# DavidHan008/SLAM-1

Measured on AMD Instinct MI355X. Metric: frames/sec tracking+local-BA @1280x720, higher is better.
Workload: dtype u8+f32+f64

## Files before the change

### slam-1_amd/csrc/ba.hip

```cpp
#include "common.hpp"

#include <cmath>

namespace {

typedef double d4 __attribute__((ext_vector_type(4)));

__device__ __forceinline__ void st_sc1(double* p, double v) {
  __hip_atomic_store(p, v, __ATOMIC_RELAXED, __HIP_MEMORY_SCOPE_AGENT);
}
__device__ __forceinline__ double ld_sc1(const double* p) {
  return __hip_atomic_load(const_cast<double*>(p), __ATOMIC_RELAXED, __HIP_MEMORY_SCOPE_AGENT);
}
__device__ __forceinline__ unsigned ticket_add(uint32_t* p) {
  return __hip_atomic_fetch_add(p, 1u, __ATOMIC_RELAXED, __HIP_MEMORY_SCOPE_AGENT);
}
__device__ __forceinline__ void ticket_reset(uint32_t* p) {
  __hip_atomic_store(p, 0u, __ATOMIC_RELAXED, __HIP_MEMORY_SCOPE_AGENT);
}

constexpr double kClamp = 5000.0;
constexpr double kDiagMin = 1e-6, kDiagMax = 1e32;
constexpr double kLamMin = 1e-16, kLamMax = 1e32;
constexpr int kBS = 256;
// ... 267 lines not shown
  if (threadIdx.x == 0) {
    const int nw = (blockDim.x + 63) >> 6;
    for (int w = 0; w < nw; ++w) s += lds[w];
  }
  __syncthreads();
  return s;
}

__global__ __launch_bounds__(kBS) void k_residual(const double* __restrict__ cams,
                                                  const double* __restrict__ pts,
                                                  const int32_t* __restrict__ ci,
                                                  const int32_t* __restrict__ pi,
                                                  const double* __restrict__ qs, int n_obs,
                                                  double* __restrict__ resid,
                                                  double* __restrict__ jac) {
  const int o = blockIdx.x * kBS + threadIdx.x;
  if (o >= n_obs) return;
  double r[2], J[2][12];
  if (jac) {
    reproject<true>(cams + 9 * ci[o], pts + 3 * pi[o], qs + 2 * o, r, J);
    clamp_rows<true>(r, J);
    for (int a = 0; a < 2; ++a)
      for (int k = 0; k < 12; ++k) jac[(size_t)o * 24 + a * 12 + k] = J[a][k];
  } else {
    reproject<false>(cams + 9 * ci[o], pts + 3 * pi[o], qs + 2 * o, r, J);
    clamp_rows<false>(r, J);
  }
  resid[2 * o] = r[0];
  resid[2 * o + 1] = r[1];
}

__device__ __forceinline__ int cur_of(const double* state) {
  return state[SLAM_BA_ST_CUR] != 0.0 ? 1 : 0;
}

__device__ __forceinline__ double clampd(double d) { return fmin(fmax(d, kDiagMin), kDiagMax); }

constexpr int kDenseMaxN = 120;
__host__ __device__ __forceinline__ bool sys_packed(int n_cams) { return 9 * n_cams > kDenseMaxN; }
__host__ __device__ __forceinline__ long long sys_vec_off(int n_cams, int n_blocks) {
  return sys_packed(n_cams) ? 81ll * n_blocks : 81ll * n_cams * n_cams;
}


struct PtSchur {
  double V00 = 0, V01 = 0, V02 = 0, V11 = 0, V12 = 0, V22 = 0, g0 = 0, g1 = 0, g2 = 0;
  double d[3], iv[6], e[3];
  __device__ __forceinline__ void acc(double j0, double j1, double j2, double rr) {
    V00 += j0 * j0; V01 += j0 * j1; V02 += j0 * j2;
    V11 += j1 * j1; V12 += j1 * j2; V22 += j2 * j2;
    g0 -= j0 * rr; g1 -= j1 * rr; g2 -= j2 * rr;
  }
  __device__ __forceinline__ void solve(double lam);
};
__device__ __forceinline__ void PtSchur::solve(double lam) {
  d[0] = clampd(V00); d[1] = clampd(V11); d[2] = clampd(V22);
  const double a00 = V00 + lam * d[0], a11 = V11 + lam * d[1], a22 = V22 + lam * d[2];
  const double a01 = V01, a02 = V02, a12 = V12;
  const double c00 = a11 * a22 - a12 * a12;
  const double c01 = a02 * a12 - a01 * a22;
  const double c02 = a01 * a12 - a02 * a11;
  const double c11 = a00 * a22 - a02 * a02;
  const double c12 = a01 * a02 - a00 * a12;
  const double c22 = a00 * a11 - a01 * a01;
  const double det = a00 * c00 + a01 * c01 + a02 * c02;
  const double id = det != 0.0 ? 1.0 / det : 0.0;
  iv[0] = c00 * id; iv[1] = c01 * id; iv[2] = c02 * id;
  iv[3] = c11 * id; iv[4] = c12 * id; iv[5] = c22 * id;
  e[0] = iv[0] * g0 + iv[1] * g1 + iv[2] * g2;
  e[1] = iv[1] * g0 + iv[3] * g1 + iv[4] * g2;
  e[2] = iv[2] * g0 + iv[4] * g1 + iv[5] * g2;
}

__device__ __forceinline__ double pt_comp(const double* jr, int stride, int kb, int ke, int j) {
  const int ia = j < 3 ? 0 : j < 5 ? 1 : j < 6 ? 2 : j - 6;
  const int ib = j < 3 ? j : j < 5 ? j - 2 : 2;
  const bool isg = j >= 6;
  const double* xr[2] = {jr + ia * stride, jr + (3 + ia) * stride};
  const double* yr[2] = {jr + (isg ? 6 : ib) * stride, jr + (isg ? 7 : 3 + ib) * stride};
  double v = 0.0;
  for (int k = kb; k < ke; k += 4) {
    double x[4][2], y[4][2];
#pragma unroll
    for (int u = 0; u < 4; ++u) {
      const int kk = min(k + u, ke - 1);
#pragma unroll
      for (int a = 0; a < 2; ++a) {
        x[u][a] = xr[a][kk];
        y[u][a] = yr[a][kk];
      }
    }
#pragma unroll
    for (int u = 0; u < 4; ++u) {
      if (k + u >= ke) break;
#pragma unroll
      for (int a = 0; a < 2; ++a) v += (isg ? -x[u][a] : x[u][a]) * y[u][a];
    }
  }
  return v;
}

constexpr int kCPart = 112;
constexpr int kGrp = 128;
constexpr int kLinWG = 256;
constexpr int kSlotLds = 128;
constexpr int kPairLds = 1024;

struct LinLds {
  double jc[kGrp][18];
  double w[kGrp][27];
  double ru[kGrp][4];
  double pt[kGrp][9];
  int lpt[kGrp];
  int cobs[kGrp];
  int cptr[kSlotLds];
  int bptr[kSlotLds];
  int pairs[kPairLds];
  unsigned fx[kGrp];
};

__device__ __forceinline__ void y_row(const double* W, const double* Vi, int i, double y[3]) {
  const double a = W[3 * i], b = W[3 * i + 1], c = W[3 * i + 2];
  y[0] = a * Vi[0] + b * Vi[1] + c * Vi[2];
  y[1] = a * Vi[1] + b * Vi[3] + c * Vi[4];
  y[2] = a * Vi[2] + b * Vi[4] + c * Vi[5];
}

__device__ __forceinline__ void lin_slots(const slam_ba_problem& p, LinLds& L, int cs0, int ncs,
                                          int bs0, int nbs, const int* cptr, int coff,
                                          const int* bptr, int boff, const int* pairs) {
  const int t = threadIdx.x;
  const int* cobs = L.cobs;
  for (int item = t; item < 9 * (ncs + nbs); item += kLinWG) {
    const int sl = item / 9, i = item - 9 * sl;
    double acc[9];
#pragma unroll
    for (int j = 0; j < 9; ++j) acc[j] = 0.0;
    if (sl < ncs) {
      const int s = cs0 + sl;
      double vr = 0.0, vu = 0.0, vd = 0.0, cost = 0.0;
      const int qb = cptr[sl] - coff, qe = cptr[sl + 1] - coff;
      int k = cobs[qb < qe ? qb : 0], lk = L.lpt[k];
      for (int q = qb; q < qe; ++q) {
        const int kn = cobs[q + 1 < qe ? q + 1 : q], lkn = L.lpt[kn];
        const double* jc = L.jc[k];
        const double* W = L.w[k];
        double y[3];
        y_row(W, L.pt[lk] + 3, i, y);
        const double a0 = jc[i], a1 = jc[9 + i];
#pragma unroll
        for (int j = 0; j < 9; ++j) {
          const double u = __builtin_fma(a0, jc[j], a1 * jc[9 + j]);
          const double v = __builtin_fma(y[0], W[3 * j], __builtin_fma(y[1], W[3 * j + 1], y[2] * W[3 * j + 2]));
          acc[j] += u - v;
        }
        const double r0 = L.ru[k][0], r1 = L.ru[k][1];
        vr = __builtin_fma(a0, r0, __builtin_fma(a1, r1, vr));
        vu = __builtin_fma(a0, L.ru[k][2], __builtin_fma(a1, L.ru[k][3], vu));
        vd = __builtin_fma(a0, a0, __builtin_fma(a1, a1, vd));
        cost = __builtin_fma(r0, r0, __builtin_fma(r1, r1, cost));
        k = kn;
        lk = lkn;
      }
      double* out = p.cpart + (size_t)p.cslot_row[s] * kCPart;
#pragma unroll
      for (int j = 0; j < 9; ++j) out[9 * i + j] = acc[j];
      out[81 + i] = vr;
      out[90 + i] = vu;
      out[99 + i] = vd;
      if (i == 0) out[108] = cost;
    } else {
      const int sb = sl - ncs, s = bs0 + sb;
      const int qb = bptr[sb] - boff, qe = bptr[sb + 1] - boff;
      int pr = pairs[qb < qe ? qb : 0], lk = L.lpt[pr & 0xffff];
      for (int q = qb; q < qe; ++q) {
        const int prn = pairs[q + 1 < qe ? q + 1 : q], lkn = L.lpt[prn & 0xffff];
        const int k1 = pr & 0xffff, k2 = pr >> 16;
        double y[3];
        y_row(L.w[k1], L.pt[lk] + 3, i, y);
        const double* W2 = L.w[k2];
#pragma unroll
        for (int j = 0; j < 9; ++j)
          acc[j] = __builtin_fma(y[0], W2[3 * j], __builtin_fma(y[1], W2[3 * j + 1], __builtin_fma(y[2], W2[3 * j + 2], acc[j])));
        pr = prn;
        lk = lkn;
      }
      double* out = p.bpart + (size_t)p.bslot_row[s] * 81;
#pragma unroll
      for (int j = 0; j < 9; ++j) out[9 * i + j] = acc[j];
    }
  }
}

#ifdef SLAM_LIN_PROFILE
#define LIN_T(i) const uint64_t lin_t##i = __builtin_amdgcn_s_memtime()
#else
#define LIN_T(i) (void)0
#endif
__global__ __launch_bounds__(kLinWG) void k_linearize(BaBatch bat) {
  BA_PROB_X(bat);
  const int g = bx;
  if (g >= p.n_grps) return;
  lm_wave_priority();
  __shared__ LinLds L;
  LIN_T(0);
  const int p0 = p.grp_ptr[g], p1 = p.grp_ptr[g + 1];
  const int o0 = p.pt_ptr[p0], o1 = p.pt_ptr[p1];
  const int t = threadIdx.x;
  const int o = o0 + t;
  const bool has = t < kGrp && o < o1;
  const int cur = cur_of(p.state);
  const int cs0 = p.grp_cslot[g], ncs = p.grp_cslot[g + 1] - cs0;
  const int bs0 = p.grp_bslot[g], nbs = p.grp_bslot[g + 1] - bs0;
  const int cb0 = p.cslot_obs_ptr[cs0], pb0 = p.bslot_pair_ptr[bs0];
  const int npairs = p.bslot_pair_ptr[bs0 + nbs] - pb0;
  const bool fit_c = ncs < kSlotLds, fit_b = nbs < kSlotLds, fit_p = npairs <= kPairLds;
  if (fit_c && t <= ncs) L.cptr[t] = p.cslot_obs_ptr[cs0 + t] - cb0;
  if (fit_b && t <= nbs) L.bptr[t] = p.bslot_pair_ptr[bs0 + t] - pb0;
  if (t < kGrp && t < o1 - o0) L.cobs[t] = p.cslot_obs[cb0 + t];
  if (fit_p)
    for (int q = t; q < npairs; q += kLinWG) L.pairs[q] = p.bslot_pairs[pb0 + q];
  double r[2], J[2][12];
  if (has) {
    const int pt = p.obs_pt[o];
    reproject_pre<true>(p.camrec[cur] + kCamRec * p.obs_cam[o], p.pts[cur] + 3 * pt,
                        p.obs_q + 2 * o, r, J);
    clamp_rows<true>(r, J);
#pragma unroll
    for (int a = 0; a < 2; ++a) {
#pragma unroll
      for (int i = 0; i < 9; ++i) L.jc[t][9 * a + i] = J[a][i];
#pragma unroll
      for (int c = 0; c < 3; ++c) L.w[t][3 * a + c] = J[a][9 + c];
      L.w[t][6 + a] = r[a];
      L.ru[t][a] = r[a];
    }
    L.lpt[t] = pt - p0;
  }
  __syncthreads();
  if (p.cam_fixed != nullptr) {
    for (int sl = t; sl < ncs; sl += kLinWG) {
      const unsigned fx = p.cam_fixed[p.cslot_cam[cs0 + sl]];
      const int qe = p.cslot_obs_ptr[cs0 + sl + 1] - cb0;
      for (int q = p.cslot_obs_ptr[cs0 + sl] - cb0; q < qe; ++q) L.fx[L.cobs[q]] = fx;
    }
    __syncthreads();
    if (has) {
      const unsigned fx = L.fx[t];
      if (fx) {
        hold_cols(J, fx);
#pragma unroll
        for (int i = 0; i < 9; ++i)
          if ((fx >> i) & 1u) L.jc[t][i] = L.jc[t][9 + i] = 0.0;
      }
    }
  }
  LIN_T(1);
  const double lam = p.state[SLAM_BA_ST_LAMBDA];
  if (t < p1 - p0) {
    const int pt = p0 + t;
    PtSchur ps;
    for (int k = p.pt_ptr[pt] - o0; k < p.pt_ptr[pt + 1] - o0; ++k) {
#pragma unroll
      for (int a = 0; a < 2; ++a) ps.acc(L.w[k][3 * a], L.w[k][3 * a + 1], L.w[k][3 * a + 2], L.w[k][6 + a]);
    }
    ps.solve(lam);
#pragma unroll
    for (int k = 0; k < 3; ++k) L.pt[t][k] = ps.e[k];
#pragma unroll
    for (int k = 0; k < 6; ++k) L.pt[t][3 + k] = ps.iv[k];
  }
  __syncthreads();
  if (has) {
    const double* e = L.pt[L.lpt[t]];
#pragma unroll
    for (int i = 0; i < 9; ++i)
#pragma unroll
      for (int c = 0; c < 3; ++c) L.w[t][3 * i + c] = J[0][i] * J[0][9 + c] + J[1][i] * J[1][9 + c];
    L.ru[t][2] = J[0][9] * e[0] + J[0][10] * e[1] + J[0][11] * e[2];
    L.ru[t][3] = J[1][9] * e[0] + J[1][10] * e[1] + J[1][11] * e[2];
  }
  __syncthreads();
  LIN_T(2);
  if (fit_c && fit_b && fit_p)
    lin_slots(p, L, cs0, ncs, bs0, nbs, L.cptr, 0, L.bptr, 0, L.pairs);
  else
    lin_slots(p, L, cs0, ncs, bs0, nbs, p.cslot_obs_ptr + cs0, cb0, p.bslot_pair_ptr + bs0, pb0,
              p.bslot_pairs + pb0);
#ifdef SLAM_LIN_PROFILE
  __builtin_amdgcn_s_waitcnt(0);
  __syncthreads();
  LIN_T(3);
  if (g == 7 && t == 0) {
    p.state[12] = (double)(lin_t1 - lin_t0);
    p.state[13] = (double)(lin_t2 - lin_t1);
    p.state[14] = (double)(lin_t3 - lin_t2);
    p.state[15] = (double)(ncs * 100 + nbs);
  }
#endif
}

constexpr int kMObs = 120, kMPts = 16, kMCams = 7, kMRows = 64;
constexpr int kMWG = 256;
constexpr int kSgMeta = 24;
constexpr int kNoObs = 255;
constexpr int kMObsS = kMObs + 1;
struct alignas(16) MLds {
  double jc[18][kMObsS];
  double jp[6][kMObsS];
  double ru[4][kMObsS];
  double vi[kMPts][6];
  double e[kMPts][3];
  double yt[kMPts][3][kMRows];
  double wt[kMPts][3][kMRows];
  double cam[kMCams][kCamRec];
  double X[kMPts][3];
  double zero;
  int optr[kMPts + 1];
  int lpt[kMObs];
  int la[kMObs];
  int cobs[kMObs];
  int cptr[8];
  uint8_t kfirst[kMPts][8];
  unsigned fx[kMCams];
  int crow[kMCams];
  int bab[kMCams * (kMCams - 1) / 2], brow[kMCams * (kMCams - 1) / 2];
};
static_assert(sizeof(MLds) <= 80 * 1024, "k_lin_mfma: two workgroups per CU");
static_assert(offsetof(MLds, ru) == offsetof(MLds, jp) + 6 * kMObsS * sizeof(double),
              "k_lin_mfma: (B) reads Jp and r as the rows of one array");
static_assert(kMObs <= kNoObs && kMCams <= 8 && kMPts * 8 <= kMWG, "k_lin_mfma: kfirst");
static_assert(16 * kMPts <= kMWG && 2 * kMCams <= 16, "k_lin_mfma: 16 lanes per point in (B), (C)");
static_assert(9 * kMCams <= kMRows, "k_lin_mfma: 9m rows in 4 tile rows");
static_assert(kMCams * kCamRec + kMCams <= kMWG, "k_lin_mfma: a lane per record entry and per mask word");
static_assert(2 * kMPts * 3 * kMRows >= kMRows * kMRows + kMCams * 256, "staging aliases yt/wt");

#ifdef SLAM_LINM_PROFILE
__device__ unsigned long long g_linm_stamp[4096][8];
#define LINM_DECL() unsigned long long linm_prev = __builtin_amdgcn_s_memtime(), linm_acc[7] = {0, 0, 0, 0, 0, 0, 0}
#define LINM_T(i)                                                  \
  do {                                                             \
    if (threadIdx.x == 0) {                                        \
      const unsigned long long linm_now = __builtin_amdgcn_s_memtime(); \
      linm_acc[i] += linm_now - linm_prev;                         \
      linm_prev = linm_now;                                        \
    }                                                              \
  } while (0)
#define LINM_END()                                                               \
  do {                                                                           \
    if (threadIdx.x == 0 && blockIdx.x + 1024 * blockIdx.y < 4096)               \
      for (int linm_i = 0; linm_i < 7; ++linm_i)                                 \
        g_linm_stamp[blockIdx.x + 1024 * blockIdx.y][linm_i] = linm_acc[linm_i]; \
  } while (0)
#else
#define LINM_DECL() (void)0
#define LINM_T(i) (void)0
#define LINM_END() (void)0
#endif

struct AsmTab {
  const int32_t* need;
  int32_t* cnt;
  const int32_t* cam_dblk;
  const int32_t* row_blk;
  int n_empty;
  const int32_t* empty;
  __device__ explicit AsmTab(const slam_ba_problem& p) {
    const int nb = p.n_blocks;
    need = p.asm_tab;
    cnt = p.asm_tab + nb;
    cam_dblk = p.asm_tab + 2 * nb;
    row_blk = cam_dblk + p.n_cams;
    n_empty = row_blk[p.n_bslots];
    empty = row_blk + p.n_bslots + 1;
  }
};

__device__ void fold_rows_sum(const double* __restrict__ part, int stride, int rb, int re, int n,
                              double* red, double* out) {
  const int t = threadIdx.x;
  const int nparts = kMWG / n, k = t / n, e = t - k * n;
  if (k < nparts) {
    double a[4] = {0.0, 0.0, 0.0, 0.0};
    int r = rb + k;
    for (; r + 3 * nparts < re; r += 4 * nparts) {
      double v[4];
#pragma unroll
      for (int u = 0; u < 4; ++u) v[u] = ld_sc1(part + (size_t)(r + u * nparts) * stride + e);
#pragma unroll
      for (int u = 0; u < 4; ++u) a[u] += v[u];
    }
    for (int u = 0; r < re; r += nparts, ++u) a[u] += ld_sc1(part + (size_t)r * stride + e);
    red[k * n + e] = (a[0] + a[1]) + (a[2] + a[3]);
  }
  __syncthreads();
  if (t < n) {
    double v = 0.0;
    for (int q = 0; q < nparts; ++q) v += red[q * n + t];
    out[t] = v;
  }
  __syncthreads();
}

__device__ void fold_block(const slam_ba_problem& p, int blk, double* scratch) {
  double* red = scratch;
  double* sh = scratch + 3 * kCPart;
  double* sb = sh + kCPart;
  const int c1 = p.blocks[2 * blk], c2 = p.blocks[2 * blk + 1];
  const int C9 = 9 * p.n_cams, t = threadIdx.x;
  double* S = p.sys;
  double* bvec = S + sys_vec_off(p.n_cams, p.n_blocks);
  double* gvec = bvec + C9;
  double* diagU = gvec + C9;
  double* costc = diagU + C9;
  const bool diag = c1 == c2;
  const int bb = p.blk_bslot_ptr[blk], be = p.blk_bslot_ptr[blk + 1];
  if (diag) fold_rows_sum(p.cpart, kCPart, p.cam_cslot_ptr[c1], p.cam_cslot_ptr[c1 + 1], 109, red, sh);
  if (be > bb) {
    fold_rows_sum(p.bpart, 81, bb, be, 81, red, sb);
  } else if (t < 81) {
    sb[t] = 0.0;
  }
  __syncthreads();
  if (sys_packed(p.n_cams)) {
    if (t < 81) S[(size_t)blk * 81 + t] = diag ? sh[t] - (sb[t] + sb[9 * (t % 9) + t / 9]) : -sb[t];
  } else if (t < 81) {
    const int i = t / 9, j = t - 9 * (t / 9);
    if (diag) {
      S[(size_t)(9 * c1 + i) * C9 + 9 * c1 + j] = sh[t] - (sb[t] + sb[9 * j + i]);
    } else {
      S[(size_t)(9 * c1 + i) * C9 + 9 * c2 + j] = -sb[t];
      S[(size_t)(9 * c2 + j) * C9 + 9 * c1 + i] = -sb[t];
    }
  }
  if (diag && t < 9) {
    gvec[9 * c1 + t] = -sh[81 + t];
    bvec[9 * c1 + t] = -sh[81 + t] - sh[90 + t];
    diagU[9 * c1 + t] = sh[99 + t];
  }
  if (diag && t == 0) costc[c1] = sh[108];
  __syncthreads();
}

__device__ void fold_zero_block(const slam_ba_problem& p, int blk, int t0, int nt) {
  const int c1 = p.blocks[2 * blk], c2 = p.blocks[2 * blk + 1];
  const int C9 = 9 * p.n_cams;
  double* S = p.sys;
  double* bvec = S + sys_vec_off(p.n_cams, p.n_blocks);
  for (int e = t0; e < 81; e += nt) {
    const int i = e / 9, j = e - 9 * (e / 9);
    if (sys_packed(p.n_cams)) {
      S[(size_t)blk * 81 + e] = 0.0;
    } else {
      S[(size_t)(9 * c1 + i) * C9 + 9 * c2 + j] = 0.0;
      S[(size_t)(9 * c2 + j) * C9 + 9 * c1 + i] = 0.0;
    }
  }
  if (c1 == c2)
    for (int e = t0; e < 28; e += nt) {
      if (e < 27) bvec[(size_t)(e / 9) * C9 + 9 * c1 + e % 9] = 0.0;
      else bvec[3 * (size_t)C9 + c1] = 0.0;
    }
}

__device__ void lin_fold_assemble(const slam_ba_problem& p, const int* cams, int m, int nb,
                                  const int* brow, double* scratch) {
  const AsmTab A(p);
  __shared__ int done[kMCams + kMCams * (kMCams - 1) / 2];
  __shared__ int ndone;
  __builtin_amdgcn_s_waitcnt(0);
  __syncthreads();
  if (threadIdx.x == 0) {
    int n = 0;
    for (int q = 0; q < m + nb; ++q) {
      const int blk = q < m ? A.cam_dblk[cams[q]] : A.row_blk[brow[q - m]];
      const int old = (int)ticket_add(reinterpret_cast<uint32_t*>(A.cnt + blk));
      if (old == A.need[blk] - 1) {
        done[n++] = blk;
        __hip_atomic_store(A.cnt + blk, 0, __ATOMIC_RELAXED, __HIP_MEMORY_SCOPE_AGENT);
      }
    }
    ndone = n;
  }
  __syncthreads();
  for (int q = 0; q < ndone; ++q) fold_block(p, done[q], scratch);
}

__global__ __launch_bounds__(kMWG) void k_lin_mfma(BaBatch bat) {
  BA_PROB_X(bat);
  const int sg = bx;
  if (sg >= p.n_sgrps) return;
  LINM_DECL();
  lm_wave_priority();
  __shared__ MLds L;
  if (p.asm_tab != nullptr) {
    const AsmTab A(p);
    for (int q = sg; q < A.n_empty; q += p.n_sgrps) fold_zero_block(p, A.empty[q], threadIdx.x, kMWG);
  }
  const int t = threadIdx.x, lane = t & 63;
  const int wid = __builtin_amdgcn_readfirstlane(t >> 6);
  const int* sm = p.sg_meta + kSgMeta * sg;
  const int ch0 = sm[0], ch1 = sm[1], cs0 = sm[2], m = sm[3], bs0 = sm[4], nb = sm[5];
  const int nt = (9 * m + 15) >> 4;
  const int cur = cur_of(p.state);
  const double lam = p.state[SLAM_BA_ST_LAMBDA];
  const bool held = p.cam_fixed != nullptr;
  if (t < kMCams * kCamRec) {
    const int a = t / kCamRec, k = t - kCamRec * (t / kCamRec);
    const int c = a < m ? sm[10 + a] : -1;
    if (c >= 0) L.cam[a][k] = p.camrec[cur][(size_t)kCamRec * c + k];
  } else if (held && t - kMCams * kCamRec < m) {
    const int a = t - kMCams * kCamRec;
    L.fx[a] = p.cam_fixed[sm[10 + a]];
  }
  if (t == 0) L.zero = 0.0;
  if (t < m) L.crow[t] = p.cslot_row[cs0 + t];
  if (t >= 64 && t - 64 < nb) {
    L.bab[t - 64] = p.bslot_ab[bs0 + t - 64];
    L.brow[t - 64] = p.bslot_row[bs0 + t - 64];
  }
  int tI[3], tJ[3];
  int ntl = 0;
  {
    int s = 0;
    for (int I = 0; I < nt; ++I)
      for (int J = I; J < nt; ++J, ++s)
        if ((s & 3) == wid && ntl < 3) {
          tI[ntl] = I;
          tJ[ntl] = J;
          ++ntl;
        }
  }
  const int nza = (m > wid) + (m > wid + 4);
  int tRow[3], tCol[3];
#pragma unroll
  for (int s = 0; s < 3; ++s) {
    tRow[s] = 16 * (s < ntl ? tI[s] : 0) + (lane & 15);
    tCol[s] = 16 * (s < ntl ? tJ[s] : 0) + (lane & 15);
  }
  d4 acc[3], zacc[2];
#pragma unroll
  for (int s = 0; s < 3; ++s) acc[s] = d4{0.0, 0.0, 0.0, 0.0};
#pragma unroll
  for (int s = 0; s < 2; ++s) zacc[s] = d4{0.0, 0.0, 0.0, 0.0};
  const int mi = lane & 15, mk = lane >> 4;

  struct ChunkIn {
    double q0, q1, xv;
    int meta, pp, cp;
  };
  auto load_in = [&](int ch, int p0, int p1, int o0, int o1) {
    ChunkIn in{0.0, 0.0, 0.0, 0, 0, 0};
    const int nobs = o1 - o0, npts = p1 - p0;
    const int ko = t & 127;
    if (ko < nobs) {
      in.q0 = p.obs_q[2 * (o0 + ko)];
      in.q1 = p.obs_q[2 * (o0 + ko) + 1];
    }
    if (t < nobs) in.meta = p.obs_meta[o0 + t];
    if (t < 3 * npts) in.xv = p.pts[cur][3 * p0 + t];
    if (t >= 128 && t - 128 <= npts) in.pp = p.pt_ptr[p0 + t - 128] - o0;
    if (t < 8) in.cp = p.chk_cptr[8 * ch + t];
    return in;
  };
  int p0 = sm[6], p1 = sm[7], o0 = sm[8], o1 = sm[9];
  int np0 = 0, np1 = 0, no0 = 0, no1 = 0;
  if (ch0 + 1 < ch1) {
    np0 = p.grp_ptr[ch0 + 1];
    np1 = p.grp_ptr[ch0 + 2];
    no0 = p.chk_optr[ch0 + 1];
    no1 = p.chk_optr[ch0 + 2];
  }
  ChunkIn in = load_in(ch0, p0, p1, o0, o1);
  {
    typedef double dbl2 __attribute__((ext_vector_type(2)));
    dbl2* y2 = reinterpret_cast<dbl2*>(&L.yt[0][0][0]);
    dbl2* w2 = reinterpret_cast<dbl2*>(&L.wt[0][0][0]);
    for (int i = t; i < kMPts * 3 * kMRows / 2; i += kMWG) {
      y2[i] = dbl2{0.0, 0.0};
      w2[i] = dbl2{0.0, 0.0};
    }
  }
  for (int ch = ch0; ch < ch1; ++ch) {
    const int nobs = o1 - o0, npts = p1 - p0;
    const double q0 = in.q0, q1 = in.q1;
    __syncthreads();
    if (t < nobs) {
      L.lpt[t] = in.meta & 255;
      L.la[t] = (in.meta >> 8) & 255;
      L.cobs[t] = in.meta >> 16;
    }
    if (t < 3 * npts) (&L.X[0][0])[t] = in.xv;
    if (t >= 128 && t - 128 <= npts) L.optr[t - 128] = in.pp;
    if (t < 8) L.cptr[t] = in.cp;
    int tl = t;
    asm volatile("" : "+v"(tl));
    if (tl < kMPts * 8) (&L.kfirst[0][0])[tl] = kNoObs;
    __syncthreads();
    if (tl < nobs && (tl == 0 || L.lpt[tl - 1] != L.lpt[tl] || L.la[tl - 1] != L.la[tl]))
      L.kfirst[L.lpt[tl]][L.la[tl]] = (uint8_t)tl;
    int nnp0 = 0, nnp1 = 0, nno0 = 0, nno1 = 0;
    if (ch + 1 < ch1) {
      in = load_in(ch + 1, np0, np1, no0, no1);
      if (ch + 2 < ch1) {
        nnp0 = p.grp_ptr[ch + 2];
        nnp1 = p.grp_ptr[ch + 3];
        nno0 = p.chk_optr[ch + 2];
        nno1 = p.chk_optr[ch + 3];
      }
    }
    LINM_T(1);
    {
      const int k = t & 127;
      if (k < nobs) {
        const double q[2] = {q0, q1};
        double r[2], Jh[2][6];
        if (t < 128) {
          reproject_half<0>(L.cam[L.la[k]], L.X[L.lpt[k]], q, r, Jh);
          if (held) hold_cols_half<0>(Jh, L.fx[L.la[k]]);
#pragma unroll
          for (int a = 0; a < 2; ++a) {
#pragma unroll
            for (int i = 0; i < 6; ++i) L.jc[9 * a + i][k] = Jh[a][i];
            L.ru[a][k] = r[a];
          }
        } else {
          reproject_half<1>(L.cam[L.la[k]], L.X[L.lpt[k]], q, r, Jh);
          if (held) hold_cols_half<1>(Jh, L.fx[L.la[k]]);
#pragma unroll
          for (int a = 0; a < 2; ++a) {
#pragma unroll
            for (int i = 0; i < 3; ++i) L.jc[9 * a + 6 + i][k] = Jh[a][i];
#pragma unroll
            for (int c = 0; c < 3; ++c) L.jp[3 * a + c][k] = Jh[a][3 + c];
          }
        }
      }
    }
    __syncthreads();
    LINM_T(2);
    {
      tl = t;
      asm volatile("" : "+v"(tl));
      const int lp = tl >> 4, j = tl & 15;
      double v = 0.0;
      if (lp < npts && j < 9) v = pt_comp(&L.jp[0][0], kMObsS, L.optr[lp], L.optr[lp + 1], j);
      PtSchur ps;
      auto row_lane = [](double x, auto sh) {
        constexpr int kSh = decltype(sh)::value;
        union { double d; int w[2]; } a, b;
        a.d = x;
        b.w[0] = __builtin_amdgcn_update_dpp(0, a.w[0], 0x100 + kSh, 0xF, 0xF, false);
        b.w[1] = __builtin_amdgcn_update_dpp(0, a.w[1], 0x100 + kSh, 0xF, 0xF, false);
        return b.d;
      };
      ps.V00 = v;
      ps.V01 = row_lane(v, std::integral_constant<int, 1>{});
      ps.V02 = row_lane(v, std::integral_constant<int, 2>{});
      ps.V11 = row_lane(v, std::integral_constant<int, 3>{});
      ps.V12 = row_lane(v, std::integral_constant<int, 4>{});
      ps.V22 = row_lane(v, std::integral_constant<int, 5>{});
      ps.g0 = row_lane(v, std::integral_constant<int, 6>{});
      ps.g1 = row_lane(v, std::integral_constant<int, 7>{});
      ps.g2 = row_lane(v, std::integral_constant<int, 8>{});
      if (lp < npts && j == 0) {
        ps.solve(lam);
#pragma unroll
        for (int k = 0; k < 3; ++k) L.e[lp][k] = ps.e[k];
#pragma unroll
        for (int k = 0; k < 6; ++k) L.vi[lp][k] = ps.iv[k];
      }
    }
    __syncthreads();
    LINM_T(3);
    {
      const int lp = tl >> 4, a = (tl & 15) >> 1, hh = tl & 1;
      if (lp < npts && a < m) {
        const int ke = L.optr[lp + 1];
        const int kf = L.kfirst[lp][a];
        const int ib = hh ? 5 : 0, ie = hh ? 9 : 5;
        const bool seen = kf != kNoObs;
        double W[5][3];
#pragma unroll
        for (int i = 0; i < 5; ++i)
#pragma unroll
          for (int c = 0; c < 3; ++c) W[i][c] = 0.0;
        for (int k = kf; k < ke && L.la[k] == a; ++k) {
#pragma unroll
          for (int i = 0; i < 5; ++i) {
            if (ib + i >= ie) break;
#pragma unroll
            for (int c = 0; c < 3; ++c)
              W[i][c] += L.jc[ib + i][k] * L.jp[c][k] + L.jc[9 + ib + i][k] * L.jp[3 + c][k];
          }
        }
        const double* vi = L.vi[lp];
        const double V[3][3] = {{vi[0], vi[1], vi[2]}, {vi[1], vi[3], vi[4]}, {vi[2], vi[4], vi[5]}};
#pragma unroll
        for (int i = 0; i < 5; ++i) {
          if (ib + i >= ie) break;
          const int row = 9 * a + ib + i;
#pragma unroll
          for (int c = 0; c < 3; ++c) {
            const int pos = (row + 16 * ((3 * lp + c) & 3)) & (kMRows - 1);
            const double y = W[i][0] * V[0][c] + W[i][1] * V[1][c] + W[i][2] * V[2][c];
            L.wt[lp][c][pos] = W[i][c];
            L.yt[lp][c][pos] = seen ? y : 0.0;
          }
        }
      }
      const int h = t >> 7, k0 = t & 127;
      if (h == 0 && k0 < nobs) {
        const double* e = L.e[L.lpt[k0]];
        L.ru[2][k0] = L.jp[0][k0] * e[0] + L.jp[1][k0] * e[1] + L.jp[2][k0] * e[2];
        L.ru[3][k0] = L.jp[3][k0] * e[0] + L.jp[4][k0] * e[1] + L.jp[5][k0] * e[2];
      }
    }
    __syncthreads();
    LINM_T(4);
    {
      const double* Yf = &L.yt[0][0][0];
      const double* Wf = &L.wt[0][0][0];
      const int nk = 3 * npts;
      for (int k0 = 0; k0 < nk; k0 += 16) {
        double av[4][3], bv[4][3];
#pragma unroll
        for (int u = 0; u < 4; ++u) {
          const int kk = min(k0 + 4 * u + mk, 3 * kMPts - 1);
#pragma unroll
          for (int s = 0; s < 3; ++s) {
            av[u][s] = Yf[kk * kMRows + ((tRow[s] + 16 * mk) & (kMRows - 1))];
            bv[u][s] = Wf[kk * kMRows + ((tCol[s] + 16 * mk) & (kMRows - 1))];
          }
        }
#pragma unroll
        for (int u = 0; u < 4; ++u) {
          const bool on = k0 + 4 * u + mk < nk;
#pragma unroll
          for (int s = 0; s < 3; ++s) {
            const bool o = on && s < ntl;
            acc[s] = __builtin_amdgcn_mfma_f64_16x16x4f64(o ? av[u][s] : 0.0, o ? bv[u][s] : 0.0,
                                                         acc[s], 0, 0, 0);
          }
        }
      }
    }
    {
      const int row = mk & 1;
      int qb[2], qe[2];
#pragma unroll
      for (int s = 0; s < 2; ++s) {
        const int a = wid + 4 * s;
        qb[s] = s < nza ? L.cptr[a] : 0;
        qe[s] = s < nza ? L.cptr[a + 1] : 0;
      }
      const int nsteps = max(qe[0] - qb[0], qe[1] - qb[1]);
      for (int q = 0; q < nsteps; q += 8) {
        double z[2][4];
        bool ok[2][4];
#pragma unroll
        for (int s = 0; s < 2; ++s)
#pragma unroll
          for (int u = 0; u < 4; ++u) {
            const int qq = qb[s] + q + 2 * u + (mk >> 1);
            ok[s][u] = qq < qe[s];
            const int k = L.cobs[ok[s][u] ? qq : 0];
            const double* src = mi < 9 ? &L.jc[9 * row + mi][k]
                                : mi < 11 ? &L.ru[row + 2 * (mi - 9)][k] : &L.zero;
            z[s][u] = *src;
          }
#pragma unroll
        for (int u = 0; u < 4; ++u)
#pragma unroll
          for (int s = 0; s < 2; ++s) {
            const double zv = ok[s][u] ? z[s][u] : 0.0;
            zacc[s] = __builtin_amdgcn_mfma_f64_16x16x4f64(zv, zv, zacc[s], 0, 0, 0);
          }
      }
    }
    p0 = np0; p1 = np1; o0 = no0; o1 = no1;
    np0 = nnp0; np1 = nnp1; no0 = nno0; no1 = nno1;
    LINM_T(5);
  }
  __syncthreads();
  double* T = &L.yt[0][0][0];
  double* Z = T + kMRows * kMRows;
#pragma unroll
  for (int s = 0; s < 3; ++s) {
    if (s >= ntl) break;
#pragma unroll
    for (int r = 0; r < 4; ++r)
      T[(16 * tI[s] + mk + 4 * r) * kMRows + 16 * tJ[s] + mi] = acc[s][r];
  }
#pragma unroll
  for (int s = 0; s < 2; ++s) {
    if (s >= nza) break;
#pragma unroll
    for (int r = 0; r < 4; ++r) Z[(wid + 4 * s) * 256 + (mk + 4 * r) * 16 + mi] = zacc[s][r];
  }
  __syncthreads();
  const bool fold = p.asm_tab != nullptr;
  for (int q = t; q < m * 109; q += kMWG) {
    const int a = q / 109, e = q - 109 * (q / 109);
    const double* Za = Z + a * 256;
    double v;
    if (e < 81) {
      const int i = e / 9, j = e - 9 * (e / 9);
      const int row = 9 * a + i, col = 9 * a + j;
      const double tv = (row >> 4) <= (col >> 4) ? T[row * kMRows + col] : T[col * kMRows + row];
      v = Za[i * 16 + j] - tv;
    } else if (e < 90) {
      v = Za[(e - 81) * 16 + 9];
    } else if (e < 99) {
      v = Za[(e - 90) * 16 + 10];
    } else if (e < 108) {
      v = Za[(e - 99) * 17];
    } else {
      v = Za[9 * 16 + 9];
    }
    double* cp = p.cpart + (size_t)L.crow[a] * kCPart + e;
    if (fold) st_sc1(cp, v);
    else *cp = v;
  }
  for (int q = t; q < 81 * nb; q += kMWG) {
    const int pr = q / 81, e = q - 81 * (q / 81);
    const int ab = L.bab[pr], a = ab & 255, b = ab >> 8;
    const int i = e / 9, j = e - 9 * (e / 9);
    const double v = T[(9 * a + i) * kMRows + 9 * b + j];
    double* bp = p.bpart + (size_t)L.brow[pr] * 81 + e;
    if (fold) st_sc1(bp, v);
    else *bp = v;
  }
  LINM_T(6);
  if (p.asm_tab != nullptr) lin_fold_assemble(p, sm + 10, m, nb, L.brow, &L.jc[0][0]);
  LINM_END();
}

#ifndef SLAM_ASM_WG
#define SLAM_ASM_WG 1024
#endif
constexpr int kAsmWG = SLAM_ASM_WG;
static_assert(kAsmWG >= 128 && kAsmWG % 64 == 0, "SLAM_ASM_WG");
__device__ void rows_sum(const double* __restrict__ part, int stride, int rb, int re, int n,
                         double (*red)[kCPart], double* out) {
  const int t = threadIdx.x;
  const int nparts = kAsmWG / n, k = t / n, e = t - k * n;
  if (k < nparts) {
    double a[8] = {0, 0, 0, 0, 0, 0, 0, 0};
    int r = rb + k;
    for (; r + 7 * nparts < re; r += 8 * nparts) {
      double v[8];
#pragma unroll
      for (int u = 0; u < 8; ++u) v[u] = part[(size_t)(r + u * nparts) * stride + e];
#pragma unroll
      for (int u = 0; u < 8; ++u) a[u] += v[u];
    }
    for (int u = 0; r < re; r += nparts, ++u) a[u] += part[(size_t)r * stride + e];
    red[k][e] = ((a[0] + a[1]) + (a[2] + a[3])) + ((a[4] + a[5]) + (a[6] + a[7]));
  }
  __syncthreads();
  if (t < n) {
    double v = 0.0;
    for (int q = 0; q < nparts; ++q) v += red[q][t];
    out[t] = v;
  }
  __syncthreads();
}

__global__ __launch_bounds__(kAsmWG) void k_assemble(BaBatch bat) {
  BA_PROB_X(bat);
  if (bx >= (p.asm_act != nullptr ? p.n_asm_act : p.n_blocks)) return;
  lm_wave_priority();
  __shared__ double red[kAsmWG / 81][kCPart];
  __shared__ double sh[kCPart];
  __shared__ double sb[81];
  const int blk = p.asm_act != nullptr ? p.asm_act[bx] : bx;
  if (p.asm_act != nullptr) {
    const int32_t* listed = p.asm_act + p.n_asm_act;
    const int32_t* camrows = listed + p.n_blocks;
    const size_t ns = (size_t)p.n_blocks * 81, c9 = 9 * (size_t)p.n_cams, nv = ns + 3 * c9 + p.n_cams;
    for (size_t i = (size_t)bx * kAsmWG + threadIdx.x; i < nv; i += (size_t)p.n_asm_act * kAsmWG) {
      if (i < ns) {
        if (!listed[i / 81]) p.sys[i] = -0.0;
      } else {
        const size_t j = i - ns;
        const int cam = j < 3 * c9 ? (int)((j % c9) / 9) : (int)(j - 3 * c9);
        if (!camrows[cam]) p.sys[i] = j < 2 * c9 ? -0.0 : 0.0;
      }
    }
  }
  const int c1 = p.blocks[2 * blk], c2 = p.blocks[2 * blk + 1];
  const int C9 = 9 * p.n_cams;
  double* S = p.sys;
  double* bvec = S + sys_vec_off(p.n_cams, p.n_blocks);
  double* gvec = bvec + C9;
  double* diagU = gvec + C9;
  double* costc = diagU + C9;
  const int t = threadIdx.x;
  const bool diag = c1 == c2;
  const int bb = p.blk_bslot_ptr[blk], be = p.blk_bslot_ptr[blk + 1];
  if (!diag && be == bb) {
    if (t < 81) {
      if (sys_packed(p.n_cams)) {
        S[(size_t)blk * 81 + t] = -0.0;
      } else {
        const int i = t / 9, j = t - 9 * (t / 9);
        S[(size_t)(9 * c1 + i) * C9 + 9 * c2 + j] = -0.0;
        S[(size_t)(9 * c2 + j) * C9 + 9 * c1 + i] = -0.0;
      }
    }
    return;
  }
  if (diag) rows_sum(p.cpart, kCPart, p.cam_cslot_ptr[c1], p.cam_cslot_ptr[c1 + 1], 109, red, sh);
  if (!diag || be > bb) {
    rows_sum(p.bpart, 81, bb, be, 81, red, sb);
  } else if (t < 81) {
    sb[t] = 0.0;
  }
  __syncthreads();
  if (sys_packed(p.n_cams)) {
    if (t < 81) S[(size_t)blk * 81 + t] = diag ? sh[t] - (sb[t] + sb[9 * (t % 9) + t / 9]) : -sb[t];
  } else if (t < 81) {
    const int i = t / 9, j = t - 9 * (t / 9);
    if (diag) {
      S[(size_t)(9 * c1 + i) * C9 + 9 * c1 + j] = sh[t] - (sb[t] + sb[9 * j + i]);
    } else {
      S[(size_t)(9 * c1 + i) * C9 + 9 * c2 + j] = -sb[t];
      S[(size_t)(9 * c2 + j) * C9 + 9 * c1 + i] = -sb[t];
    }
  }
  if (diag && t < 9) {
    gvec[9 * c1 + t] = -sh[81 + t];
    bvec[9 * c1 + t] = -sh[81 + t] - sh[90 + t];
    diagU[9 * c1 + t] = sh[99 + t];
  }
  if (diag && t == 0) costc[c1] = sh[108];
}

constexpr int kLdsMaxN = kDenseMaxN;
constexpr int kSolveHdr = 32;

struct EpiSrc {
  const double *g, *dU, *cam, *costc;
};
#ifdef SLAM_FLOW_PROFILE
__device__ unsigned long long g_flow_epi[4];
#endif

__device__ __forceinline__ void block_sum2(double& a, double& b, double* lds) {
  for (int off = 32; off > 0; off >>= 1) {
    a += __shfl_down(a, off, 64);
    b += __shfl_down(b, off, 64);
  }
  const int lane = threadIdx.x & 63, wid = threadIdx.x >> 6;
  if (lane == 0) {
    lds[wid] = a;
    lds[16 + wid] = b;
  }
  __syncthreads();
  if (threadIdx.x == 0) {
    const int nw = (blockDim.x + 63) >> 6;
    a = 0.0;
    b = 0.0;
    for (int w = 0; w < nw; ++w) {
      a += lds[w];
      b += lds[16 + w];
    }
  }
  __syncthreads();
}

template <bool GLOBAL = false>
__device__ void solve_epilogue(const slam_ba_problem& p, const double* x, bool ok, double* red,
                               const EpiSrc& e, int fail_code = 1) {
  const int C9 = 9 * p.n_cams, t = threadIdx.x;
  double* state = p.state;
  const double lam = state[SLAM_BA_ST_LAMBDA];
  const int cur = cur_of(state);
  double pc = 0.0, cost = 0.0;
  if constexpr (GLOBAL) {
    const int nt = blockDim.x;
    for (int i0 = t; i0 < C9; i0 += 8 * nt) {
      double xv[8], cv[8], uv[8], gv[8];
#pragma unroll
      for (int q = 0; q < 8; ++q) {
        const int i = min(i0 + q * nt, C9 - 1);
        xv[q] = x[i];
        cv[q] = e.cam[i];
        uv[q] = e.dU[i];
        gv[q] = e.g[i];
      }
#pragma unroll
      for (int q = 0; q < 8; ++q) {
        const int i = i0 + q * nt;
        if (i < C9) {
          const double d = ok ? xv[q] : 0.0;
          p.delta_c[i] = d;
          p.cams[1 - cur][i] = cv[q] + d;
          pc += d * (lam * clampd(uv[q]) * d + gv[q]);
        }
      }
    }
    for (int c = t; c < p.n_cams; c += nt) cost += e.costc[c];
    block_sum2(pc, cost, red);
#ifdef SLAM_FLOW_PROFILE
    if (t == 0) g_flow_epi[2] = wall_clock64();
#endif
  } else {
    for (int i = t; i < C9; i += blockDim.x) {
      const double d = ok ? x[i] : 0.0;
      p.delta_c[i] = d;
      p.cams[1 - cur][i] = e.cam[i] + d;
      pc += d * (lam * clampd(e.dU[i]) * d + e.g[i]);
    }
    pc = block_sum(pc, red);
    if (t == 0)
      for (int c = 0; c < p.n_cams; ++c) cost += e.costc[c];
  }
  for (int c = t; c < p.n_cams; c += blockDim.x)
    cam_prep(p.cams[1 - cur] + 9 * c, p.camrec[1 - cur] + kCamRec * c);
#ifdef SLAM_FLOW_PROFILE
  if (GLOBAL) {
    __builtin_amdgcn_s_waitcnt(0);
    __syncthreads();
    if (t == 0) g_flow_epi[3] = wall_clock64();
  }
#endif
  if (t == 0) {
    state[SLAM_BA_ST_COST] = 0.5 * cost;
    state[SLAM_BA_ST_PRED_CAM] = 0.5 * pc;
    state[SLAM_BA_ST_CHOL_FAIL] = ok ? 0.0 : (double)fail_code;
    if (!ok && fail_code == 2) state[SLAM_BA_ST_SOLVE_FAULT] += 1.0;
  }
}

#ifdef SLAM_SOLVE_PROFILE
#define SOLVE_PROF_T(i) uint64_t prof_t##i = wall_clock64()
#define SOLVE_PROF_END()                                                        \
  do {                                                                          \
    const uint64_t prof_e = wall_clock64();                                     \
    if (threadIdx.x == 0) {                                                     \
      p.state[12] = 10.0 * (double)(prof_t1 - prof_t0);                         \
      p.state[13] = 10.0 * (double)(prof_t2 - prof_t1);                         \
      p.state[14] = 10.0 * (double)(prof_t3 - prof_t2);                         \
      p.state[15] = 10.0 * (double)(prof_e - prof_t3);                          \
    }                                                                           \
  } while (0)
#else
#define SOLVE_PROF_T(i) (void)0
#define SOLVE_PROF_END() (void)0
#endif

constexpr int kBlkWG = 256;
constexpr int kBlkWaves = kBlkWG / 64;
constexpr int kTileMax = 9;
constexpr int kPanelW = 9;
constexpr int kWLs = 13;
static_assert(kLdsMaxN <= kBlkWG, "k_solve_blk prefetch assumes one element per thread");
static_assert(kBlkWaves * kTileMax >= ((kLdsMaxN + 16) / 16) * ((kLdsMaxN + 16) / 16 + 1) / 2,
              "kTileMax too small");

__device__ __forceinline__ double rcp_f64(double d) {
  double r = __builtin_amdgcn_rcp(d);
  double e = __builtin_fma(-d, r, 1.0);
  r = __builtin_fma(r, e, r);
  e = __builtin_fma(-d, r, 1.0);
  return __builtin_fma(r, e, r);
}

__device__ __forceinline__ double readlane_d(double v, int lane) {
  const unsigned long long u = (unsigned long long)__double_as_longlong(v);
  const unsigned lo = (unsigned)__builtin_amdgcn_readlane((int)(unsigned)u, lane);
  const unsigned hi = (unsigned)__builtin_amdgcn_readlane((int)(unsigned)(u >> 32), lane);
  return __longlong_as_double((long long)(((unsigned long long)hi << 32) | lo));
}

struct BlkLds {
  int n16;
  int pn, wl, ll, lf, dd, yy, xx, ep, total;
  __host__ __device__ explicit BlkLds(int n) {
    n16 = ((n + 1 + 15) / 16) * 16;
    pn = kSolveHdr;
    wl = pn + n16 * kPanelW;
    ll = wl + n16 * kWLs;
    lf = ll + n16 * kWLs;
    dd = lf + ((n * (n - 1) / 2 + 1) & ~1);
    yy = dd + ((n + 1) & ~1);
    xx = yy + ((n + 1) & ~1);
    ep = xx + ((n + 1) & ~1);
    total = ep + 5 * ((n + 1) & ~1);
  }
};

#ifdef SLAM_SOLVE_TRACE
__device__ unsigned long long g_solve_trace[20][6];
#define SOLVE_TR(step, i)                                                        \
  do {                                                                           \
    if (threadIdx.x == 0 && blockIdx.y == 0 && (step) < 20)                      \
      g_solve_trace[step][i] = __builtin_amdgcn_s_memtime();                     \
  } while (0)
#else
// ... 2403 lines not shown
```

Before: 22700.

## Rebalance Schur tile and camera-block MFMA work across waves with static deal

Replaces the round-robin assignment of upper-triangular Schur tiles and camera blocks to waves with a fixed per-wave deal table, balancing MFMA load. One wave gets three tiles in a shared row, so it loads a single A operand for all three. The inner loops are specialised by template on tile and camera counts, dropping the per-iteration masking of unused tiles. The LDS struct is reordered and the per-wave accumulators are merged into one array of five. This adds code-size and register pressure from the template variants, and it hardcodes the layout for up to 7 cameras and 4 waves.

Result: faster. 22980 (median of 6 runs) (+1.2%).

```diff
diff --git a/slam-1_amd/csrc/ba.hip b/slam-1_amd/csrc/ba.hip
--- a/slam-1_amd/csrc/ba.hip
+++ b/slam-1_amd/csrc/ba.hip
@@ -593,17 +593,13 @@
 
 constexpr int kMObs = 120, kMPts = 16, kMCams = 7, kMRows = 64;
 constexpr int kMWG = 256;
+constexpr int kFoldWG = 256;
 constexpr int kSgMeta = 24;
 constexpr int kNoObs = 255;
 constexpr int kMObsS = kMObs + 1;
 struct alignas(16) MLds {
-  double jc[18][kMObsS];
-  double jp[6][kMObsS];
-  double ru[4][kMObsS];
   double vi[kMPts][6];
   double e[kMPts][3];
-  double yt[kMPts][3][kMRows];
-  double wt[kMPts][3][kMRows];
   double cam[kMCams][kCamRec];
   double X[kMPts][3];
   double zero;
@@ -616,30 +612,46 @@
   unsigned fx[kMCams];
   int crow[kMCams];
   int bab[kMCams * (kMCams - 1) / 2], brow[kMCams * (kMCams - 1) / 2];
+  alignas(8) double jc[18][kMObsS];
+  double jp[6][kMObsS];
+  double ru[4][kMObsS];
+  alignas(16) double yt[kMPts][3][kMRows];
+  double wt[kMPts][3][kMRows];
 };
 static_assert(sizeof(MLds) <= 80 * 1024, "k_lin_mfma: two workgroups per CU");
 static_assert(offsetof(MLds, ru) == offsetof(MLds, jp) + 6 * kMObsS * sizeof(double),
               "k_lin_mfma: (B) reads Jp and r as the rows of one array");
 static_assert(kMObs <= kNoObs && kMCams <= 8 && kMPts * 8 <= kMWG, "k_lin_mfma: kfirst");
 static_assert(16 * kMPts <= kMWG && 2 * kMCams <= 16, "k_lin_mfma: 16 lanes per point in (B), (C)");
+static_assert(kMWG == 256 && kMCams <= 7 && kMRows == 64, "k_lin_mfma: the deal of (D) covers 4 waves, 10 tiles and 7 cameras");
 static_assert(9 * kMCams <= kMRows, "k_lin_mfma: 9m rows in 4 tile rows");
 static_assert(kMCams * kCamRec + kMCams <= kMWG, "k_lin_mfma: a lane per record entry and per mask word");
-static_assert(2 * kMPts * 3 * kMRows >= kMRows * kMRows + kMCams * 256, "staging aliases yt/wt");
+static_assert(2 * kMPts * 3 * kMRows >= kMRows * kMRows + kMCams * 256 &&
+                  offsetof(MLds, wt) == offsetof(MLds, yt) + sizeof(MLds::yt),
+              "staging aliases yt/wt");
 
 #ifdef SLAM_LINM_PROFILE
+#ifndef SLAM_LINM_WAVE
+#define SLAM_LINM_WAVE 0
+#endif
+#define LINM_ON (threadIdx.x == 64 * SLAM_LINM_WAVE)
 __device__ unsigned long long g_linm_stamp[4096][8];
-#define LINM_DECL() unsigned long long linm_prev = __builtin_amdgcn_s_memtime(), linm_acc[7] = {0, 0, 0, 0, 0, 0, 0}
-#define LINM_T(i)                                                  \
-  do {                                                             \
-    if (threadIdx.x == 0) {                                        \
+#define LINM_DECL()                                            \
+  __shared__ unsigned long long linm_acc[7];                   \
+  unsigned long long linm_prev = __builtin_amdgcn_s_memtime(); \
+  if (LINM_ON)                                                 \
+    for (int linm_i = 0; linm_i < 7; ++linm_i) linm_acc[linm_i] = 0
+#define LINM_T(i)                                                       \
+  do {                                                                  \
+    if (LINM_ON) {                                                      \
       const unsigned long long linm_now = __builtin_amdgcn_s_memtime(); \
-      linm_acc[i] += linm_now - linm_prev;                         \
-      linm_prev = linm_now;                                        \
-    }                                                              \
+      linm_acc[i] += linm_now - linm_prev;                              \
+      linm_prev = linm_now;                                             \
+    }                                                                   \
   } while (0)
 #define LINM_END()                                                               \
   do {                                                                           \
-    if (threadIdx.x == 0 && blockIdx.x + 1024 * blockIdx.y < 4096)               \
+    if (LINM_ON && blockIdx.x + 1024 * blockIdx.y < 4096)                        \
       for (int linm_i = 0; linm_i < 7; ++linm_i)                                 \
         g_linm_stamp[blockIdx.x + 1024 * blockIdx.y][linm_i] = linm_acc[linm_i]; \
   } while (0)
@@ -670,7 +682,7 @@
 __device__ void fold_rows_sum(const double* __restrict__ part, int stride, int rb, int re, int n,
                               double* red, double* out) {
   const int t = threadIdx.x;
-  const int nparts = kMWG / n, k = t / n, e = t - k * n;
+  const int nparts = kFoldWG / n, k = t / n, e = t - k * n;
   if (k < nparts) {
     double a[4] = {0.0, 0.0, 0.0, 0.0};
     int r = rb + k;
@@ -777,6 +789,78 @@
   for (int q = 0; q < ndone; ++q) fold_block(p, done[q], scratch);
 }
 
+constexpr unsigned kDealI[3] = {0x2010u, 0x2210u, 0x2310u};
+constexpr unsigned kDealJ[3] = {0x2310u, 0xF321u, 0xF332u};
+constexpr unsigned kDealC[3] = {0x0235u, 0x1FF6u, 0x4FFFu};
+
+template <int NTL, bool SHJ>
+__device__ __forceinline__ void linm_schur(const MLds& L, d4 (&u)[5], int nk, const int (&I)[3],
+                                           const int (&J)[3], int lane) {
+  const double* Yf = &L.yt[0][0][0];
+  const double* Wf = &L.wt[0][0][0];
+  const int mi = lane & 15, mk = lane >> 4;
+  constexpr int NA = SHJ ? NTL : 1, NB = SHJ ? 1 : NTL;
+  int ra[NA], rb[NB];
+#pragma unroll
+  for (int s = 0; s < NA; ++s) ra[s] = (16 * I[s] + mi + 16 * mk) & (kMRows - 1);
+#pragma unroll
+  for (int s = 0; s < NB; ++s) rb[s] = (16 * J[s] + mi + 16 * mk) & (kMRows - 1);
+  for (int k0 = 0; k0 < nk; k0 += 16) {
+    double av[4][NA], bv[4][NB];
+#pragma unroll
+    for (int v = 0; v < 4; ++v) {
+      const int kk = min(k0 + 4 * v + mk, 3 * kMPts - 1);
+#pragma unroll
+      for (int s = 0; s < NA; ++s) av[v][s] = Yf[kk * kMRows + ra[s]];
+#pragma unroll
+      for (int s = 0; s < NB; ++s) bv[v][s] = Wf[kk * kMRows + rb[s]];
+    }
+#pragma unroll
+    for (int v = 0; v < 4; ++v) {
+      const bool on = k0 + 4 * v + mk < nk;
+#pragma unroll
+      for (int s = 0; s < NTL; ++s)
+        u[s] = __builtin_amdgcn_mfma_f64_16x16x4f64(on ? av[v][SHJ ? s : 0] : 0.0, on ? bv[v][SHJ ? 0 : s] : 0.0,
+                                                    u[s], 0, 0, 0);
+    }
+  }
+}
+
+template <int B0, int NZA>
+__device__ __forceinline__ void linm_cams(const MLds& L, d4 (&u)[5], const int (&cam)[3], int lane) {
+  const int mi = lane & 15, mk = lane >> 4, row = mk & 1;
+  int qb[NZA], qe[NZA];
+  int nsteps = 0;
+#pragma unroll
+  for (int s = 0; s < NZA; ++s) {
+    qb[s] = __builtin_amdgcn_readfirstlane(L.cptr[cam[s]]);
+    qe[s] = __builtin_amdgcn_readfirstlane(L.cptr[cam[s] + 1]);
+    nsteps = max(nsteps, qe[s] - qb[s]);
+  }
+  for (int q = 0; q < nsteps; q += 8) {
+    double z[NZA][4];
+    bool ok[NZA][4];
+#pragma unroll
+    for (int s = 0; s < NZA; ++s)
+#pragma unroll
+      for (int v = 0; v < 4; ++v) {
+        const int qq = qb[s] + q + 2 * v + (mk >> 1);
+        ok[s][v] = qq < qe[s];
+        const int k = L.cobs[ok[s][v] ? qq : 0];
+        const double* src = mi < 9 ? &L.jc[9 * row + mi][k]
+                            : mi < 11 ? &L.ru[row + 2 * (mi - 9)][k] : &L.zero;
+        z[s][v] = *src;
+      }
+#pragma unroll
+    for (int v = 0; v < 4; ++v)
+#pragma unroll
+      for (int s = 0; s < NZA; ++s) {
+        const double zv = ok[s][v] ? z[s][v] : 0.0;
+        u[B0 + s] = __builtin_amdgcn_mfma_f64_16x16x4f64(zv, zv, u[B0 + s], 0, 0, 0);
+      }
+  }
+}
+
 __global__ __launch_bounds__(kMWG) void k_lin_mfma(BaBatch bat) {
   BA_PROB_X(bat);
   const int sg = bx;
@@ -810,37 +894,29 @@
     L.bab[t - 64] = p.bslot_ab[bs0 + t - 64];
     L.brow[t - 64] = p.bslot_row[bs0 + t - 64];
   }
-  int tI[3], tJ[3];
-  int ntl = 0;
-  {
-    int s = 0;
-    for (int I = 0; I < nt; ++I)
-      for (int J = I; J < nt; ++J, ++s)
-        if ((s & 3) == wid && ntl < 3) {
-          tI[ntl] = I;
-          tJ[ntl] = J;
-          ++ntl;
-        }
-  }
-  const int nza = (m > wid) + (m > wid + 4);
-  int tRow[3], tCol[3];
+  int tI[3], tJ[3], zc[3];
+  int ntl = 0, nza = 0;
 #pragma unroll
   for (int s = 0; s < 3; ++s) {
-    tRow[s] = 16 * (s < ntl ? tI[s] : 0) + (lane & 15);
-    tCol[s] = 16 * (s < ntl ? tJ[s] : 0) + (lane & 15);
-  }
-  d4 acc[3], zacc[2];
-#pragma unroll
-  for (int s = 0; s < 3; ++s) acc[s] = d4{0.0, 0.0, 0.0, 0.0};
-#pragma unroll
-  for (int s = 0; s < 2; ++s) zacc[s] = d4{0.0, 0.0, 0.0, 0.0};
+    tI[s] = (kDealI[s] >> (4 * wid)) & 15;
+    tJ[s] = (kDealJ[s] >> (4 * wid)) & 15;
+    ntl += tJ[s] < nt;
+  }
+#pragma unroll
+  for (int s = 0; s < 3; ++s) {
+    zc[s] = (kDealC[s] >> (4 * wid)) & 15;
+    nza += zc[s] < m;
+  }
+  d4 acc[5];
+#pragma unroll
+  for (int s = 0; s < 5; ++s) acc[s] = d4{0.0, 0.0, 0.0, 0.0};
   const int mi = lane & 15, mk = lane >> 4;
 
   struct ChunkIn {
     double q0, q1, xv;
     int meta, pp, cp;
   };
-  auto load_in = [&](int ch, int p0, int p1, int o0, int o1) {
+  auto load_in = [&](int t, int ch, int p0, int p1, int o0, int o1) {
     ChunkIn in{0.0, 0.0, 0.0, 0, 0, 0};
     const int nobs = o1 - o0, npts = p1 - p0;
     const int ko = t & 127;
@@ -862,7 +938,7 @@
     no0 = p.chk_optr[ch0 + 1];
     no1 = p.chk_optr[ch0 + 2];
   }
-  ChunkIn in = load_in(ch0, p0, p1, o0, o1);
+  ChunkIn in = load_in(t, ch0, p0, p1, o0, o1);
   {
     typedef double dbl2 __attribute__((ext_vector_type(2)));
     dbl2* y2 = reinterpret_cast<dbl2*>(&L.yt[0][0][0]);
@@ -876,23 +952,23 @@
     const int nobs = o1 - o0, npts = p1 - p0;
     const double q0 = in.q0, q1 = in.q1;
     __syncthreads();
-    if (t < nobs) {
-      L.lpt[t] = in.meta & 255;
-      L.la[t] = (in.meta >> 8) & 255;
-      L.cobs[t] = in.meta >> 16;
-    }
-    if (t < 3 * npts) (&L.X[0][0])[t] = in.xv;
-    if (t >= 128 && t - 128 <= npts) L.optr[t - 128] = in.pp;
-    if (t < 8) L.cptr[t] = in.cp;
     int tl = t;
     asm volatile("" : "+v"(tl));
+    if (tl < nobs) {
+      L.lpt[tl] = in.meta & 255;
+      L.la[tl] = (in.meta >> 8) & 255;
+      L.cobs[tl] = in.meta >> 16;
+    }
+    if (tl < 3 * npts) (&L.X[0][0])[tl] = in.xv;
+    if (tl >= 128 && tl - 128 <= npts) L.optr[tl - 128] = in.pp;
+    if (tl < 8) L.cptr[tl] = in.cp;
     if (tl < kMPts * 8) (&L.kfirst[0][0])[tl] = kNoObs;
     __syncthreads();
     if (tl < nobs && (tl == 0 || L.lpt[tl - 1] != L.lpt[tl] || L.la[tl - 1] != L.la[tl]))
       L.kfirst[L.lpt[tl]][L.la[tl]] = (uint8_t)tl;
     int nnp0 = 0, nnp1 = 0, nno0 = 0, nno1 = 0;
     if (ch + 1 < ch1) {
-      in = load_in(ch + 1, np0, np1, no0, no1);
+      in = load_in(tl, ch + 1, np0, np1, no0, no1);
       if (ch + 2 < ch1) {
         nnp0 = p.grp_ptr[ch + 2];
         nnp1 = p.grp_ptr[ch + 3];
@@ -902,7 +978,7 @@
     }
     LINM_T(1);
     {
-      const int k = t & 127;
+      const int k = tl & 127;
       if (k < nobs) {
         const double q[2] = {q0, q1};
         double r[2], Jh[2][6];
@@ -1010,63 +1086,26 @@
     __syncthreads();
     LINM_T(4);
     {
-      const double* Yf = &L.yt[0][0][0];
-      const double* Wf = &L.wt[0][0][0];
       const int nk = 3 * npts;
-      for (int k0 = 0; k0 < nk; k0 += 16) {
-        double av[4][3], bv[4][3];
-#pragma unroll
-        for (int u = 0; u < 4; ++u) {
-          const int kk = min(k0 + 4 * u + mk, 3 * kMPts - 1);
-#pragma unroll
-          for (int s = 0; s < 3; ++s) {
-            av[u][s] = Yf[kk * kMRows + ((tRow[s] + 16 * mk) & (kMRows - 1))];
-            bv[u][s] = Wf[kk * kMRows + ((tCol[s] + 16 * mk) & (kMRows - 1))];
-          }
-        }
-#pragma unroll
-        for (int u = 0; u < 4; ++u) {
-          const bool on = k0 + 4 * u + mk < nk;
-#pragma unroll
-          for (int s = 0; s < 3; ++s) {
-            const bool o = on && s < ntl;
-            acc[s] = __builtin_amdgcn_mfma_f64_16x16x4f64(o ? av[u][s] : 0.0, o ? bv[u][s] : 0.0,
-                                                         acc[s], 0, 0, 0);
-          }
-        }
-      }
-    }
-    {
-      const int row = mk & 1;
-      int qb[2], qe[2];
-#pragma unroll
-      for (int s = 0; s < 2; ++s) {
-        const int a = wid + 4 * s;
-        qb[s] = s < nza ? L.cptr[a] : 0;
-        qe[s] = s < nza ? L.cptr[a + 1] : 0;
-      }
-      const int nsteps = max(qe[0] - qb[0], qe[1] - qb[1]);
-      for (int q = 0; q < nsteps; q += 8) {
-        double z[2][4];
-        bool ok[2][4];
-#pragma unroll
-        for (int s = 0; s < 2; ++s)
-#pragma unroll
-          for (int u = 0; u < 4; ++u) {
-            const int qq = qb[s] + q + 2 * u + (mk >> 1);
-            ok[s][u] = qq < qe[s];
-            const int k = L.cobs[ok[s][u] ? qq : 0];
-            const double* src = mi < 9 ? &L.jc[9 * row + mi][k]
-                                : mi < 11 ? &L.ru[row + 2 * (mi - 9)][k] : &L.zero;
-            z[s][u] = *src;
-          }
-#pragma unroll
-        for (int u = 0; u < 4; ++u)
-#pragma unroll
-          for (int s = 0; s < 2; ++s) {
-            const double zv = ok[s][u] ? z[s][u] : 0.0;
-            zacc[s] = __builtin_amdgcn_mfma_f64_16x16x4f64(zv, zv, zacc[s], 0, 0, 0);
-          }
+      int ld = lane;
+      asm volatile("" : "+v"(ld));
+      if (wid == 2) {
+        if (ntl == 3) linm_schur<3, true>(L, acc, nk, tI, tJ, ld);
+      } else if (ntl == 3) {
+        linm_schur<3, false>(L, acc, nk, tI, tJ, ld);
+      } else if (ntl == 2) {
+        linm_schur<2, false>(L, acc, nk, tI, tJ, ld);
+      } else if (ntl == 1) {
+        linm_schur<1, false>(L, acc, nk, tI, tJ, ld);
+      }
+      if (wid == 3) {
+        if (nza == 3) linm_cams<1, 3>(L, acc, zc, ld);
+        else if (nza == 2) linm_cams<1, 2>(L, acc, zc, ld);
+        else if (nza == 1) linm_cams<1, 1>(L, acc, zc, ld);
+      } else if (nza == 2) {
+        linm_cams<3, 2>(L, acc, zc, ld);
+      } else if (nza == 1) {
+        linm_cams<3, 1>(L, acc, zc, ld);
       }
     }
     p0 = np0; p1 = np1; o0 = no0; o1 = no1;
@@ -1077,17 +1116,18 @@
   double* T = &L.yt[0][0][0];
   double* Z = T + kMRows * kMRows;
 #pragma unroll
-  for (int s = 0; s < 3; ++s) {
-    if (s >= ntl) break;
-#pragma unroll
-    for (int r = 0; r < 4; ++r)
-      T[(16 * tI[s] + mk + 4 * r) * kMRows + 16 * tJ[s] + mi] = acc[s][r];
-  }
-#pragma unroll
-  for (int s = 0; s < 2; ++s) {
-    if (s >= nza) break;
-#pragma unroll
-    for (int r = 0; r < 4; ++r) Z[(wid + 4 * s) * 256 + (mk + 4 * r) * 16 + mi] = zacc[s][r];
+  for (int s = 0; s < 5; ++s) {
+    const int ts = wid == 3 ? (s == 0 ? 0 : 3) : s;
+    const int zs = wid == 3 ? s - 1 : s - 3;
+    if (ts < 3 && ts < ntl) {
+      const int I = ts == 0 ? tI[0] : ts == 1 ? tI[1] : tI[2], J = ts == 0 ? tJ[0] : ts == 1 ? tJ[1] : tJ[2];
+#pragma unroll
+      for (int r = 0; r < 4; ++r) T[(16 * I + mk + 4 * r) * kMRows + 16 * J + mi] = acc[s][r];
+    } else if (zs >= 0 && zs < nza) {
+      const int a = zs == 0 ? zc[0] : zs == 1 ? zc[1] : zc[2];
+#pragma unroll
+      for (int r = 0; r < 4; ++r) Z[a * 256 + (mk + 4 * r) * 16 + mi] = acc[s][r];
+    }
   }
   __syncthreads();
   const bool fold = p.asm_tab != nullptr;
```
